# quadjr/aframe-gaussian-splatting

Measured on NVIDIA H100. Metric: frames/sec @1920x1080 (sort + splat raster, 1 M synthetic train-like splats), higher is better.
Workload: dtype f64 sort keys + f32 shading

## Files before the change

aframe-gaussian-splatting_b200/csrc/gs_sort.cu:

```cuda
#include <type_traits>

#include "gs_common.cuh"
#include "gs_depthkey.cuh"

namespace gs {

__device__ __forceinline__ bool worker_keep(const SortConsts &sc, const float4 c, const float s, double &depth) {
  const double x = c.x, y = c.y, z = c.z;
  depth = __dadd_rn(__dadd_rn(__dadd_rn(__dmul_rn(sc.view[0], x), __dmul_rn(sc.view[1], y)), __dmul_rn(sc.view[2], z)),
                    sc.view[3]);
  bool in_box = true;
  if (sc.has_cutout) {
    const double *e = sc.cutout;
    const double ny = -y;
    const double w = __ddiv_rn(
        1.0, __dadd_rn(__dadd_rn(__dadd_rn(__dmul_rn(e[3], x), __dmul_rn(e[7], ny)), __dmul_rn(e[11], z)), e[15]));
    const double c0 = __dmul_rn(
        __dadd_rn(__dadd_rn(__dadd_rn(__dmul_rn(e[0], x), __dmul_rn(e[4], ny)), __dmul_rn(e[8], z)), e[12]), w);
    const double c1 = __dmul_rn(
        __dadd_rn(__dadd_rn(__dadd_rn(__dmul_rn(e[1], x), __dmul_rn(e[5], ny)), __dmul_rn(e[9], z)), e[13]), w);
    const double c2 = __dmul_rn(
        __dadd_rn(__dadd_rn(__dadd_rn(__dmul_rn(e[2], x), __dmul_rn(e[6], ny)), __dmul_rn(e[10], z)), e[14]), w);
    if (c0 < -0.5 || c0 > 0.5 || c1 < -0.5 || c1 > 0.5 || c2 < -0.5 || c2 > 0.5) in_box = false;
  }
  return (depth < 0.0) && ((double)s > __dmul_rn(-0.0001, depth)) && in_box;
}

__global__ void __launch_bounds__(256) k_depth_cull(const float4 *__restrict__ cs, const float *__restrict__ sa,
                                                    const FrameParams *__restrict__ fp,
                                                    float *__restrict__ depth_out, FrameCounters *ctr) {
  GS_PDL_ENTRY();
  const SortConsts sc = fp->sc;
  const uint32_t n = fp->n_splats;
  double dmin = INFINITY, dmax = -INFINITY;
  uint32_t cnt = 0;
  const uint32_t stride = gridDim.x * blockDim.x;
  auto process = [&](uint32_t i, const float4 c, const float s) {
    double depth;
    const bool keep = worker_keep(sc, c, s, depth);
    float out = GS_DEPTH_REJECT;
    if (keep) {
      out = (float)depth;
      ++cnt;
      if (depth > dmax) dmax = depth;
      if (depth < dmin) dmin = depth;
    }
    depth_out[i] = out;
  };
  for (uint32_t i = blockIdx.x * blockDim.x + threadIdx.x; i < n; i += 2 * stride) {
    const uint32_t j = i + stride;
    const bool two = j < n;
    const float4 c0 = __ldg(cs + i);
    const float s0 = __ldg(sa + i);
    float4 c1 = c0;
    float s1 = s0;
    if (two) {
      c1 = __ldg(cs + j);
      s1 = __ldg(sa + j);
    }
    process(i, c0, s0);
    if (two) process(j, c1, s1);
  }
  for (int o = 16; o > 0; o >>= 1) {
    const double a = __shfl_xor_sync(0xffffffffu, dmin, o);
    const double b = __shfl_xor_sync(0xffffffffu, dmax, o);
    dmin = a < dmin ? a : dmin;
    dmax = b > dmax ? b : dmax;
    cnt += __shfl_xor_sync(0xffffffffu, cnt, o);
  }
  __shared__ double s_min[8], s_max[8];
  __shared__ uint32_t s_cnt[8];
  const int w = threadIdx.x >> 5, l = threadIdx.x & 31;
  if (l == 0) { s_min[w] = dmin; s_max[w] = dmax; s_cnt[w] = cnt; }
  __syncthreads();
  if (threadIdx.x == 0) {
    for (int k = 1; k < 8; ++k) {
      if (s_min[k] < dmin) dmin = s_min[k];
      if (s_max[k] > dmax) dmax = s_max[k];
      cnt += s_cnt[k];
    }
    if (cnt) {
      atomicMax(&ctr->sort.min_enc, ~enc_f64(dmin));
      atomicMax(&ctr->sort.max_enc, enc_f64(dmax));
      atomicAdd(&ctr->sort.n_valid, cnt);
    }
  }
}

__global__ void __launch_bounds__(256) k_depth_cull_scene(const float4 *__restrict__ cs, const float *__restrict__ sa,
                                                          const FrameParams *__restrict__ fp, const SceneTable *__restrict__ scene,
                                                          float *__restrict__ depth_out, FrameCounters *ctr, ObjCounters *octr) {
  GS_PDL_ENTRY();
  __shared__ uint32_t s_first[kMaxObjects], s_end[kMaxObjects], s_cnt[kMaxObjects];
  __shared__ unsigned long long s_min[kMaxObjects], s_max[kMaxObjects];
  const uint32_t n_obj = scene->n;
  for (uint32_t k = threadIdx.x; k < n_obj; k += blockDim.x) {
    s_first[k] = scene->obj[k].first;
    s_end[k] = scene->obj[k].end;
    s_cnt[k] = 0;
    s_min[k] = 0;
    s_max[k] = 0;
  }
  __syncthreads();
  const uint32_t n = fp->n_splats;
  const uint32_t stride = gridDim.x * blockDim.x;
  int cur = -1;
  double dmin = INFINITY, dmax = -INFINITY;
  uint32_t cnt = 0;
  auto flush = [&]() {
    if (cnt) {
      atomicMax(&s_min[cur], ~enc_f64(dmin));
      atomicMax(&s_max[cur], enc_f64(dmax));
      atomicAdd(&s_cnt[cur], cnt);
    }
    dmin = INFINITY;
    dmax = -INFINITY;
    cnt = 0;
  };
  auto process = [&](uint32_t i, const float4 c, const float s) {
    float out = GS_DEPTH_REJECT;
    const int k = scene_find(s_first, s_end, n_obj, i);
    double depth;
    if (k >= 0 && worker_keep(scene->obj[k].sc, c, s, depth)) {
      if (k != cur) {
        flush();
        cur = k;
      }
      out = (float)depth;
      ++cnt;
      if (depth > dmax) dmax = depth;
      if (depth < dmin) dmin = depth;
    }
    depth_out[i] = out;
  };
  for (uint32_t i = blockIdx.x * blockDim.x + threadIdx.x; i < n; i += 2 * stride) {
    const uint32_t j = i + stride;
    const bool two = j < n;
    const float4 c0 = __ldg(cs + i);
    const float s0 = __ldg(sa + i);
    float4 c1 = c0;
    float s1 = s0;
    if (two) {
      c1 = __ldg(cs + j);
      s1 = __ldg(sa + j);
    }
    process(i, c0, s0);
    if (two) process(j, c1, s1);
  }
  flush();
  __syncthreads();
  for (uint32_t k = threadIdx.x; k < n_obj; k += blockDim.x) {
    if (!s_cnt[k]) continue;
    atomicMax(&octr[k].min_enc, s_min[k]);
    atomicMax(&octr[k].max_enc, s_max[k]);
    atomicAdd(&octr[k].n_valid, s_cnt[k]);
    atomicMax(&ctr->sort.min_enc, s_min[k]);
    atomicMax(&ctr->sort.max_enc, s_max[k]);
    atomicAdd(&ctr->sort.n_valid, s_cnt[k]);
  }
}

template <bool IL>
__global__ void __launch_bounds__(256) k_scene_keys(const float *__restrict__ depth, const FrameParams *__restrict__ fp,
                                                    const SceneTable *__restrict__ scene, const ObjCounters *__restrict__ octr,
                                                    FrameCounters *ctr, uint32_t *__restrict__ key_out,
                                                    uint32_t *__restrict__ pay_out) {
  GS_PDL_ENTRY();
  __shared__ SceneKeyTable s_ent;
  __shared__ uint32_t s_in, s_drop;
  s_ent.load<IL>(scene, octr, ctr);
  if (threadIdx.x == 0) { s_in = 0; s_drop = 0; }
  __syncthreads();
  const uint32_t n = ctr->sort.n_valid ? fp->n_splats : 0u;
  uint32_t in = 0, drop = 0;
  for (uint32_t i = blockIdx.x * blockDim.x + threadIdx.x; i < n; i += gridDim.x * blockDim.x) {
    const float d = __ldg(depth + i);
    uint32_t key = kNoKey;
    if (d != GS_DEPTH_REJECT) {
      int k;
      key = s_ent.key<IL>(i, d, k);
      if (!IL && (key & 65536u)) {
        pay_out[i] = s_ent.first[k];
        ++drop;
      } else {
        pay_out[i] = i;
        ++in;
      }
    }
    key_out[i] = key;
  }
  for (int o = 16; o > 0; o >>= 1) {
    in += __shfl_xor_sync(0xffffffffu, in, o);
    drop += __shfl_xor_sync(0xffffffffu, drop, o);
  }
  if ((threadIdx.x & 31u) == 0) {
    if (in) atomicAdd(&s_in, in);
    if (drop) atomicAdd(&s_drop, drop);
  }
  __syncthreads();
  if (threadIdx.x == 0) {
    if (s_in) atomicAdd(&ctr->sort.n_inrange, s_in);
    if (s_drop) atomicAdd(&ctr->sort.n_dropped, s_drop);
  }
}

static int persistent_grid(gs_context *c, uint64_t n_elems, int per_cta, int ctas_per_sm) {
  uint64_t tiles = (n_elems + per_cta - 1) / per_cta;
  uint64_t cap = (uint64_t)c->sm_count * ctas_per_sm;
  if (tiles < 1) tiles = 1;
  return (int)(tiles < cap ? tiles : cap);
}

void launch_depth_cull(gs_context *c, const FrameParams *fp, FrameCounters *ctr, cudaStream_t st) {
  const int grid = persistent_grid(c, c->cap, 256 * 4, 8);
  launch_chain(c, k_depth_cull, grid, 256, st, c->center_scale, c->size_alpha, fp, c->depth, ctr);
}

void launch_depth_cull_scene(gs_context *c, const FrameParams *fp, const SceneTable *scene, ObjCounters *octr, FrameCounters *ctr,
                             cudaStream_t st) {
  const int grid = persistent_grid(c, c->cap, 256 * 4, 8);
  launch_chain(c, k_depth_cull_scene, grid, 256, st, c->center_scale, c->size_alpha, fp, scene, c->depth, ctr, octr);
}

void launch_scene_keys(gs_context *c, const FrameParams *fp, const SceneTable *scene, const ObjCounters *octr, FrameCounters *ctr,
                       bool interleave, cudaStream_t st) {
  const int grid = persistent_grid(c, c->cap, 256 * 4, 8);
  launch_chain(c, interleave ? k_scene_keys<true> : k_scene_keys<false>, grid, 256, st, (const float *)c->depth, fp, scene, octr,
               ctr, c->scene_key, c->scene_pay);
}

struct RadixScratch {
  uint32_t *table;
  uint32_t *totals;
  uint32_t stride;
};

struct RadixPass {
  using Carry = void;
  __device__ void prepare(uint32_t n) {}
  __device__ void hist_prologue(uint32_t n) const {}
  __device__ void hist_epilogue() {}
  __device__ void scanned(uint32_t total) const {}
  __device__ void digit_range(uint32_t d, uint32_t start, uint32_t end) const {}
};

template <class Pass>
__global__ void __launch_bounds__(kRadixThreads) k_radix_hist(Pass p, const RadixScratch s) {
  GS_PDL_ENTRY();
  __shared__ uint32_t h[256];
  const uint32_t tid = threadIdx.x, lane = tid & 31, warp = tid >> 5;
  const uint32_t n = p.count();
  const uint32_t num_chunks = (n + kRadixTile - 1) / kRadixTile;
  p.prepare(n);
  p.hist_prologue(n);
  for (uint32_t c = blockIdx.x; c < num_chunks; c += gridDim.x) {
    h[tid] = 0;
    __syncthreads();
    const uint32_t base = c * kRadixTile + warp * (32 * kRadixItems) + lane;
#pragma unroll
    for (int k = 0; k < kRadixItems; ++k) {
      const uint32_t i = base + k * 32;
      if (i < n) {
        uint32_t pay, carry;
        const uint32_t digit = p.load(i, pay, carry);
        if (digit != kInvalidDigit) atomicAdd(&h[digit], 1u);
      }
    }
    __syncthreads();
    s.table[(size_t)tid * s.stride + c] = h[tid];
    __syncthreads();
  }
  p.hist_epilogue();
}

template <class Pass>
__global__ void __launch_bounds__(256) k_radix_scan(const Pass p, const RadixScratch s) {
  GS_PDL_ENTRY();
  __shared__ uint32_t s_warp[8];
  __shared__ uint32_t s_carry;
  const uint32_t tid = threadIdx.x, lane = tid & 31, warp = tid >> 5;
  const uint32_t n = p.count();
  const uint32_t num_chunks = (n + kRadixTile - 1) / kRadixTile;
  uint32_t *row = s.table + (size_t)blockIdx.x * s.stride;
  if (tid == 0) s_carry = 0;
  __syncthreads();
  for (uint32_t b = 0; b < num_chunks; b += 256) {
    const uint32_t i = b + tid;
    const uint32_t v = (i < num_chunks) ? row[i] : 0u;
    uint32_t incl = v;
    for (int o = 1; o < 32; o <<= 1) {
      const uint32_t t = __shfl_up_sync(0xffffffffu, incl, o);
      if (lane >= (uint32_t)o) incl += t;
    }
    if (lane == 31) s_warp[warp] = incl;
    __syncthreads();
    uint32_t wbase = 0;
    for (uint32_t k = 0; k < warp; ++k) wbase += s_warp[k];
    const uint32_t carry = s_carry;
    if (i < num_chunks) row[i] = carry + wbase + incl - v;
    __syncthreads();
    if (tid == 255) s_carry = carry + wbase + incl;
    __syncthreads();
  }
  if (tid == 0) {
    s.totals[blockIdx.x] = s_carry;
    p.scanned(s_carry);
  }
}

constexpr int kScatThreads = 512;
constexpr int kScatItems = kRadixTile / kScatThreads;
constexpr int kScatWarps = kScatThreads / 32;

template <class Pass>
__global__ void __launch_bounds__(kScatThreads, 2) k_radix_scatter(Pass p, const RadixScratch s) {
  GS_PDL_ENTRY();
  constexpr bool kCarry = !std::is_void<typename Pass::Carry>::value;
  using carry_t = typename std::conditional<kCarry, typename Pass::Carry, uint8_t>::type;
  __shared__ uint32_t wcnt[kScatWarps][256];
  __shared__ uint32_t tile_off[256];
  __shared__ uint32_t s_loc[256];
  __shared__ uint32_t s_warp_tot[8];
  __shared__ uint32_t s_pay[kRadixTile];
  __shared__ carry_t s_carry[kCarry ? kRadixTile : 1];
  __shared__ uint8_t s_dig[kRadixTile];
  __shared__ uint32_t s_total;
  const uint32_t tid = threadIdx.x, lane = tid & 31, warp = tid >> 5;
  const uint32_t n = p.count();
  const uint32_t num_chunks = (n + kRadixTile - 1) / kRadixTile;
  if (blockIdx.x >= num_chunks) return;

  auto scan256 = [&](uint32_t v) -> uint32_t {
    uint32_t incl = v;
    for (int o = 1; o < 32; o <<= 1) {
      const uint32_t t = __shfl_up_sync(0xffffffffu, incl, o);
      if (lane >= (uint32_t)o) incl += t;
    }
    __syncthreads();
    if (lane == 31 && warp < 8) s_warp_tot[warp] = incl;
    __syncthreads();
    uint32_t wbase = 0;
    for (uint32_t k = 0; k < warp && k < 8; ++k) wbase += s_warp_tot[k];
    return wbase + incl - v;
  };

  const uint32_t dtot = tid < 256 ? s.totals[tid] : 0u;
  const uint32_t dbase = scan256(dtot);
  if (blockIdx.x == 0 && tid < 256) p.digit_range(tid, dbase, dbase + dtot);
  p.prepare(n);

  for (uint32_t c = blockIdx.x; c < num_chunks; c += gridDim.x) {
    const uint32_t toff = tid < 256 ? __ldg(s.table + (size_t)tid * s.stride + c) : 0u;
    for (uint32_t k = tid; k < kScatWarps * 256; k += kScatThreads) (&wcnt[0][0])[k] = 0u;
    const uint32_t base = c * kRadixTile + warp * (32 * kScatItems) + lane;
    uint32_t digit[kScatItems], pay[kScatItems], rank[kScatItems];
    carry_t carry[kScatItems];
#pragma unroll
    for (int k = 0; k < kScatItems; ++k) {
      const uint32_t i = base + k * 32;
      uint32_t cv = 0;
      digit[k] = kInvalidDigit;
      pay[k] = 0;
      if (i < n) digit[k] = p.load(i, pay[k], cv);
      carry[k] = (carry_t)cv;
    }
    __syncthreads();
#pragma unroll
    for (int k = 0; k < kScatItems; ++k) {
      const uint32_t d = digit[k];
      const uint32_t peers = __match_any_sync(0xffffffffu, d);
      const uint32_t lt = __popc(peers & ((1u << lane) - 1u));
      uint32_t prior = 0;
      if (d != kInvalidDigit) prior = wcnt[warp][d];
      __syncwarp();
      if (d != kInvalidDigit && lt == 0) wcnt[warp][d] = prior + __popc(peers);
      __syncwarp();
      rank[k] = prior + lt;
    }
    __syncthreads();
    uint32_t total = 0;
    if (tid < 256) {
#pragma unroll
      for (int w = 0; w < kScatWarps; ++w) {
        const uint32_t cnt = wcnt[w][tid];
        wcnt[w][tid] = total;
        total += cnt;
      }
    }
    const uint32_t loc = scan256(total);
    if (tid < 256) {
      s_loc[tid] = loc;
      tile_off[tid] = dbase + toff - loc;
      if (tid == 255) s_total = loc + total;
    }
    __syncthreads();
#pragma unroll
    for (int k = 0; k < kScatItems; ++k) {
      const uint32_t d = digit[k];
      if (d == kInvalidDigit) continue;
      const uint32_t lp = s_loc[d] + wcnt[warp][d] + rank[k];
      s_pay[lp] = pay[k];
      s_dig[lp] = (uint8_t)d;
      if (kCarry) s_carry[lp] = carry[k];
    }
    __syncthreads();
    const uint32_t nvalid = s_total;
    for (uint32_t i = tid; i < nvalid; i += kScatThreads)
      p.store(tile_off[s_dig[i]] + i, s_pay[i], kCarry ? (uint32_t)s_carry[i] : 0u);
    __syncthreads();
  }
}

template <class Pass>
static void run_pass(gs_context *c, const Pass &p, const RadixScratch &s, uint64_t n_max, cudaStream_t st) {
  const int grid = persistent_grid(c, n_max, kRadixTile, 8);
  launch_chain(c, k_radix_hist<Pass>, grid, kRadixThreads, st, p, s);
  launch_chain(c, k_radix_scan<Pass>, 256, 256, st, p, s);
  launch_chain(c, k_radix_scatter<Pass>, grid, kScatThreads, st, p, s);
}

struct D1 : RadixPass {
  using Carry = uint8_t;
  FrameCounters *ctr;
  const FrameParams *fp;
  const float *depth;
  uint32_t *idx_out; uint8_t *hi_out;
  DepthRange dr;
  uint32_t n_in, n_drop;
  __device__ uint32_t count() const { return ctr->sort.n_valid ? fp->n_splats : 0u; }
  __device__ void prepare(uint32_t n) { if (n) dr = load_depth_range(ctr); }
  __device__ uint32_t load(uint32_t i, uint32_t &pay, uint32_t &carry) {
    const float d = __ldg(depth + i);
    if (d == GS_DEPTH_REJECT) return kInvalidDigit;
    const int32_t key = depth_key(d, dr.min_depth, dr.depth_inv);
    if (key < 0 || key > 65535) { ++n_drop; return kInvalidDigit; }
    ++n_in;
    pay = i;
    carry = (uint32_t)key >> 8;
    return key & 255;
  }
  __device__ void store(uint32_t pos, uint32_t pay, uint32_t carry) const { idx_out[pos] = pay; hi_out[pos] = (uint8_t)carry; }
  __device__ void hist_epilogue() {
    __shared__ uint32_t s_in, s_drop;
    uint32_t in = n_in, drop = n_drop;
    for (int o = 16; o > 0; o >>= 1) {
      in += __shfl_xor_sync(0xffffffffu, in, o);
      drop += __shfl_xor_sync(0xffffffffu, drop, o);
    }
    if (threadIdx.x == 0) { s_in = 0; s_drop = 0; }
    __syncthreads();
    if ((threadIdx.x & 31u) == 0) { if (in) atomicAdd(&s_in, in); if (drop) atomicAdd(&s_drop, drop); }
    __syncthreads();
    if (threadIdx.x == 0) {
      if (s_in) atomicAdd(&ctr->sort.n_inrange, s_in);
      if (s_drop) atomicAdd(&ctr->sort.n_dropped, s_drop);
    }
  }
};

struct D2 : RadixPass {
  const FrameCounters *ctr;
  const uint8_t *dig; const uint32_t *idx;
  uint32_t *order;
  __device__ uint32_t count() const { return ctr->sort.n_inrange; }
  __device__ void hist_prologue(uint32_t n) const {
    const uint32_t nv = ctr->sort.n_valid;
    for (uint32_t j = n + blockIdx.x * blockDim.x + threadIdx.x; j < nv; j += gridDim.x * blockDim.x) order[j] = 0u;
  }
  __device__ uint32_t load(uint32_t i, uint32_t &pay, uint32_t &) const { pay = idx[i]; return dig[i]; }
  __device__ void store(uint32_t pos, uint32_t pay, uint32_t) const { order[pos] = pay; }
};

void launch_depth_radix(gs_context *c, const FrameParams *fp, FrameCounters *ctr, const FrameBufs &b, cudaStream_t st) {
  const RadixScratch s{c->table_n, c->totals, c->table_n_stride};
  run_pass(c, D1{{}, ctr, fp, c->depth, c->idx_a, c->dig_a}, s, c->cap, st);
  run_pass(c, D2{{}, ctr, c->dig_a, c->idx_a, b.order}, s, c->cap, st);
}

struct M1 : RadixPass {
  using Carry = uint16_t;
  const FrameCounters *ctr;
  const FrameParams *fp;
  const uint32_t *key, *pay_in;
  uint32_t *idx_out; uint16_t *hi_out;
  __device__ uint32_t count() const { return ctr->sort.n_valid ? fp->n_splats : 0u; }
  __device__ uint32_t load(uint32_t i, uint32_t &pay, uint32_t &carry) const {
    const uint32_t k = key[i];
    if (k == kNoKey) return kInvalidDigit;
    carry = k >> 8;
    pay = pay_in[i];
    return k & 255u;
  }
  __device__ void store(uint32_t pos, uint32_t pay, uint32_t carry) const { idx_out[pos] = pay; hi_out[pos] = (uint16_t)carry; }
};

struct M2 : RadixPass {
  using Carry = uint8_t;
  const FrameCounters *ctr;
  const uint16_t *hi; const uint32_t *idx;
  uint32_t *idx_out; uint8_t *hi_out;
  __device__ uint32_t count() const { return ctr->sort.n_valid; }
  __device__ uint32_t load(uint32_t i, uint32_t &pay, uint32_t &carry) const {
    const uint32_t h = hi[i];
    carry = h >> 8;
    pay = idx[i];
    return h & 255u;
  }
  __device__ void store(uint32_t pos, uint32_t pay, uint32_t carry) const { idx_out[pos] = pay; hi_out[pos] = (uint8_t)carry; }
};

struct M3 : RadixPass {
  const FrameCounters *ctr;
  const uint8_t *dig; const uint32_t *idx;
  uint32_t *order;
  __device__ uint32_t count() const { return ctr->sort.n_valid; }
  __device__ uint32_t load(uint32_t i, uint32_t &pay, uint32_t &) const { pay = idx[i]; return dig[i]; }
  __device__ void store(uint32_t pos, uint32_t pay, uint32_t) const { order[pos] = pay; }
};

void launch_scene_radix(gs_context *c, const FrameParams *fp, FrameCounters *ctr, const FrameBufs &b, cudaStream_t st) {
  const RadixScratch s{c->table_n, c->totals, c->table_n_stride};
  run_pass(c, M1{{}, ctr, fp, c->scene_key, c->scene_pay, c->idx_a, c->scene_hi}, s, c->cap, st);
  run_pass(c, M2{{}, ctr, c->scene_hi, c->idx_a, c->scene_pay, c->dig_a}, s, c->cap, st);
  run_pass(c, M3{{}, ctr, c->dig_a, c->scene_pay, b.order}, s, c->cap, st);
}

struct S1 : RadixPass {
  using Carry = uint8_t;
  const FrameCounters *ctr;
  const uint16_t *key; const uint32_t *idx;
  uint32_t *idx_out; uint8_t *hi_out;
  __device__ uint32_t count() const { return ctr->sort.n_valid; }
  __device__ uint32_t load(uint32_t i, uint32_t &pay, uint32_t &carry) const {
    const uint32_t k = key[i];
    carry = k >> 8;
    pay = idx[i];
    return k & 255u;
  }
  __device__ void store(uint32_t pos, uint32_t pay, uint32_t carry) const { idx_out[pos] = pay; hi_out[pos] = (uint8_t)carry; }
};

struct SM1 : RadixPass {
  using Carry = uint16_t;
  const FrameCounters *ctr;
  const SceneTable *scene;
  const uint32_t *key, *idx;
  uint32_t *idx_out; uint16_t *hi_out;
  __device__ uint32_t count() const { return ctr->sort.n_valid; }
  __device__ uint32_t load(uint32_t i, uint32_t &pay, uint32_t &carry) const {
    const uint32_t k = key[i];
    carry = k >> 8;
    pay = idx[i];
    if (k & 65536u) {
      uint32_t lo = 0, hi = scene->n;
      while (hi - lo > 1) {
        const uint32_t mid = (lo + hi) >> 1;
        if (scene->obj[mid].first <= pay) lo = mid; else hi = mid;
      }
      pay = scene->obj[lo].first;
    }
    return k & 255u;
  }
  __device__ void store(uint32_t pos, uint32_t pay, uint32_t carry) const { idx_out[pos] = pay; hi_out[pos] = (uint16_t)carry; }
};

struct SM1I : SM1 {
  __device__ uint32_t load(uint32_t i, uint32_t &pay, uint32_t &carry) const {
    const uint32_t k = key[i];
    carry = k >> 8;
    pay = idx[i];
    return k & 255u;
  }
};

void launch_slab_sort(gs_context *c, const FrameParams *fp, FrameCounters *ctr, const SceneTable *scene, bool interleave,
                      const FrameBufs &b, cudaStream_t st) {
  const RadixScratch s{c->table_n, c->totals, c->table_n_stride};
  if (scene) {
    const SM1 p1{{}, ctr, scene, c->scene_key, c->cidx, c->idx_a, c->scene_hi};
    if (interleave) run_pass(c, SM1I{p1}, s, c->cap, st);
    else run_pass(c, p1, s, c->cap, st);
    run_pass(c, M2{{}, ctr, c->scene_hi, c->idx_a, c->scene_pay, c->dig_a}, s, c->cap, st);
    run_pass(c, M3{{}, ctr, c->dig_a, c->scene_pay, b.order}, s, c->cap, st);
    return;
  }
  run_pass(c, S1{{}, ctr, c->ckey, c->cidx, c->idx_a, c->dig_a}, s, c->cap, st);
  run_pass(c, D2{{}, ctr, c->dig_a, c->idx_a, b.order}, s, c->cap, st);
}

__device__ __forceinline__ uint32_t f32_key(float d) { return ~__float_as_uint(d); }

__device__ __forceinline__ uint32_t scene_rank(const SceneTable *__restrict__ scene, uint32_t s) {
  uint32_t lo = 0, hi = scene->n;
  while (hi - lo > 1) {
    const uint32_t mid = (lo + hi) >> 1;
    if (scene->obj[mid].first <= s) lo = mid; else hi = mid;
  }
  return scene->obj[lo].rank;
}

constexpr int kRankDigit = -1;
template <int kShift, bool kAll>
struct Z : RadixPass {
  FrameCounters *ctr;
  const FrameParams *fp;
  const SceneTable *scene;
  const float *depth;
  const uint32_t *idx;
  uint32_t *idx_out;
  __device__ uint32_t count() const { return kAll ? (ctr->sort.n_valid ? fp->n_splats : 0u) : ctr->sort.n_valid; }
  __device__ uint32_t load(uint32_t i, uint32_t &pay, uint32_t &) const {
    const uint32_t s = kAll ? i : idx[i];
    pay = s;
    if constexpr (kShift == kRankDigit) {
      if (kAll && __ldg(depth + s) == GS_DEPTH_REJECT) return kInvalidDigit;
      return scene_rank(scene, s);
    } else {
      const float d = __ldg(depth + s);
      if (kAll && d == GS_DEPTH_REJECT) return kInvalidDigit;
      return (f32_key(d) >> kShift) & 255u;
    }
  }
  __device__ void store(uint32_t pos, uint32_t pay, uint32_t) const { idx_out[pos] = pay; }
  __device__ void scanned(uint32_t total) const {
    if (kAll && total) atomicAdd(&ctr->sort.n_inrange, total);
  }
};

template <bool kAll>
static void sort_f32(gs_context *c, const FrameParams *fp, FrameCounters *ctr, const SceneTable *scene, bool interleave,
                     const float *depth, const uint32_t *src, uint32_t *order, cudaStream_t st) {
  const RadixScratch s{c->table_n, c->totals, c->table_n_stride};
  uint32_t *a = c->idx_a, *b = c->scene_pay;
  if (scene && interleave) {
    run_pass(c, Z<kRankDigit, kAll>{{}, ctr, fp, scene, depth, src, a}, s, c->cap, st);
    run_pass(c, Z<0, false>{{}, ctr, fp, scene, depth, a, b}, s, c->cap, st);
    run_pass(c, Z<8, false>{{}, ctr, fp, scene, depth, b, a}, s, c->cap, st);
    run_pass(c, Z<16, false>{{}, ctr, fp, scene, depth, a, b}, s, c->cap, st);
    run_pass(c, Z<24, false>{{}, ctr, fp, scene, depth, b, order}, s, c->cap, st);
    return;
  }
  run_pass(c, Z<0, kAll>{{}, ctr, fp, scene, depth, src, a}, s, c->cap, st);
  run_pass(c, Z<8, false>{{}, ctr, fp, scene, depth, a, b}, s, c->cap, st);
  run_pass(c, Z<16, false>{{}, ctr, fp, scene, depth, b, a}, s, c->cap, st);
  if (!scene) {
    run_pass(c, Z<24, false>{{}, ctr, fp, scene, depth, a, order}, s, c->cap, st);
    return;
  }
  run_pass(c, Z<24, false>{{}, ctr, fp, scene, depth, a, b}, s, c->cap, st);
  run_pass(c, Z<kRankDigit, false>{{}, ctr, fp, scene, depth, b, order}, s, c->cap, st);
}

void launch_sort_f32(gs_context *c, const FrameParams *fp, FrameCounters *ctr, const SceneTable *scene, bool interleave,
                     const FrameBufs &b, cudaStream_t st) {
  sort_f32<true>(c, fp, ctr, scene, interleave, c->depth, nullptr, b.order, st);
}

void launch_slab_sort_f32(gs_context *c, FrameCounters *ctr, const SceneTable *scene, bool interleave, const float *zdepth,
                          const FrameBufs &b, cudaStream_t st) {
  sort_f32<false>(c, nullptr, ctr, scene, interleave, zdepth, c->cidx, b.order, st);
}

__device__ __forceinline__ void gather_record(const float4 *rec, float4 *inst_rec, uint32_t splat, uint32_t pos) {
  const float4 r0 = __ldg(rec + 2 * (size_t)splat);
  const float4 r1 = __ldg(rec + 2 * (size_t)splat + 1);
  inst_rec[2 * (size_t)pos] = r0;
  inst_rec[2 * (size_t)pos + 1] = r1;
}

struct T1 : RadixPass {
  using Carry = uint16_t;
  FrameCounters *ctr;
  const uint16_t *bin; const uint32_t *idx;
  uint16_t *bin_out; uint32_t *idx_out;
  const float4 *proj_rec; float4 *inst_rec; uint2 *bin_range;
  uint32_t n_bins;
  bool last;
  __device__ uint32_t count() const { return ctr->overflow ? 0u : (uint32_t)ctr->n_inst; }
  __device__ uint32_t load(uint32_t i, uint32_t &pay, uint32_t &carry) const {
    const uint16_t t = bin[i];
    if (t == kNoTile) return kInvalidDigit;
    carry = t;
    pay = idx[i];
    return t & 255;
  }
  __device__ void store(uint32_t pos, uint32_t pay, uint32_t carry) const {
    if (last) gather_record(proj_rec, inst_rec, pay, pos);
    else { idx_out[pos] = pay; bin_out[pos] = (uint16_t)carry; }
  }
  __device__ void scanned(uint32_t total) const { if (total) atomicAdd(&ctr->n_inst_kept, total); }
  __device__ void digit_range(uint32_t d, uint32_t start, uint32_t end) const {
    if (last && d < n_bins) bin_range[d] = make_uint2(start, end);
  }
};

struct T2 : RadixPass {
  using Carry = uint16_t;
  const FrameCounters *ctr;
  const uint16_t *bin; const uint32_t *idx;
  const float4 *proj_rec; float4 *inst_rec; uint16_t *bin_out;
  __device__ uint32_t count() const { return ctr->overflow ? 0u : ctr->n_inst_kept; }
  __device__ uint32_t load(uint32_t i, uint32_t &pay, uint32_t &carry) const {
    const uint16_t t = bin[i];
    carry = t;
    pay = idx[i];
    return (uint32_t)t >> 8;
  }
  __device__ void store(uint32_t pos, uint32_t pay, uint32_t carry) const {
    gather_record(proj_rec, inst_rec, pay, pos);
    bin_out[pos] = (uint16_t)carry;
  }
};

__global__ void __launch_bounds__(256) k_tile_ranges(const uint16_t *__restrict__ tile_f, FrameCounters *ctr,
                                                     uint2 *__restrict__ range) {
  GS_PDL_ENTRY();
  const uint32_t n = ctr->overflow ? 0u : ctr->n_inst_kept;
  for (uint32_t i = blockIdx.x * blockDim.x + threadIdx.x; i < n; i += gridDim.x * blockDim.x) {
    const uint32_t t = tile_f[i];
    if (i == 0 || tile_f[i - 1] != t) range[t].x = i;
    if (i == n - 1 || tile_f[i + 1] != t) range[t].y = i + 1;
  }
}

struct ViewRecs {
  const float4 *rec_x;
  uint32_t x_stride;
  uint32_t base1, base2, base3;
  __device__ __forceinline__ const float4 *of(const float4 *rec0, uint32_t bin) const {
    const uint32_t v = (bin >= base1 ? 1u : 0u) + (bin >= base2 ? 1u : 0u) + (bin >= base3 ? 1u : 0u);
    return v ? rec_x + 2 * (size_t)(v - 1) * x_stride : rec0;
  }
};
struct T1S : T1 {
  ViewRecs vr;
  __device__ void store(uint32_t pos, uint32_t pay, uint32_t carry) const {
    if (last) gather_record(vr.of(proj_rec, carry), inst_rec, pay, pos);
    else { idx_out[pos] = pay; bin_out[pos] = (uint16_t)carry; }
  }
};
struct T2S : T2 {
  ViewRecs vr;
  __device__ void store(uint32_t pos, uint32_t pay, uint32_t carry) const {
    gather_record(vr.of(proj_rec, carry), inst_rec, pay, pos);
    bin_out[pos] = (uint16_t)carry;
  }
};

struct T1P : T1 {
  uint32_t *pay_out;
  __device__ void store(uint32_t pos, uint32_t pay, uint32_t carry) const {
    if (last) { gather_record(proj_rec, inst_rec, pay, pos); pay_out[pos] = pay; }
    else { idx_out[pos] = pay; bin_out[pos] = (uint16_t)carry; }
  }
};
struct T2P : T2 {
  uint32_t *pay_out;
  __device__ void store(uint32_t pos, uint32_t pay, uint32_t carry) const {
    gather_record(proj_rec, inst_rec, pay, pos);
    pay_out[pos] = pay;
    bin_out[pos] = (uint16_t)carry;
  }
};

void launch_tile_radix_pick(gs_context *c, FrameCounters *ctr, const FrameBufs &b, uint32_t n_bins, uint32_t *pay, cudaStream_t st) {
  const RadixScratch s{c->table_d, c->totals + 256, c->table_d_stride};
  const bool last = n_bins <= 256u;
  const T1 t1{{}, ctr, c->inst_tile, c->inst_idx, c->inst_tile_b, c->inst_idx_b, b.proj_rec, b.inst_rec, b.bin_range, n_bins, last};
  run_pass(c, T1P{t1, pay}, s, c->cap_inst, st);
  if (last) return;
  const T2 t2{{}, ctr, c->inst_tile_b, c->inst_idx_b, b.proj_rec, b.inst_rec, c->inst_tile_f};
  run_pass(c, T2P{t2, pay}, s, c->cap_inst, st);
  launch_chain(c, k_tile_ranges, persistent_grid(c, c->cap_inst, 256 * 8, 8), 256, st, (const uint16_t *)c->inst_tile_f, ctr,
               b.bin_range);
}

void launch_tile_radix(gs_context *c, FrameCounters *ctr, const FrameBufs &b, uint32_t n_bins, cudaStream_t st) {
  const RadixScratch s{c->table_d, c->totals + 256, c->table_d_stride};
  const bool last = n_bins <= 256u;
  if (b.views) {
    static_assert(kMaxViews == 4, "ViewRecs holds three bases");
    const ViewRecs vr{b.proj_recx, b.x_stride, b.bin_base[1], b.bin_base[2], b.bin_base[3]};
    const T1 t1{{}, ctr, c->inst_tile, c->inst_idx, c->inst_tile_b, c->inst_idx_b, b.proj_rec, b.inst_rec, b.bin_range, n_bins, last};
    run_pass(c, T1S{t1, vr}, s, c->cap_inst, st);
    if (last) return;
    const T2 t2{{}, ctr, c->inst_tile_b, c->inst_idx_b, b.proj_rec, b.inst_rec, c->inst_tile_f};
    run_pass(c, T2S{t2, vr}, s, c->cap_inst, st);
    launch_chain(c, k_tile_ranges, persistent_grid(c, c->cap_inst, 256 * 8, 8), 256, st, (const uint16_t *)c->inst_tile_f, ctr,
                 b.bin_range);
    return;
  }
  run_pass(c, T1{{}, ctr, c->inst_tile, c->inst_idx, c->inst_tile_b, c->inst_idx_b, b.proj_rec, b.inst_rec, b.bin_range, n_bins, last},
           s, c->cap_inst, st);
  if (last) return;
  run_pass(c, T2{{}, ctr, c->inst_tile_b, c->inst_idx_b, b.proj_rec, b.inst_rec, c->inst_tile_f}, s, c->cap_inst, st);
  launch_chain(c, k_tile_ranges, persistent_grid(c, c->cap_inst, 256 * 8, 8), 256, st, (const uint16_t *)c->inst_tile_f, ctr,
               b.bin_range);
}

template <int kShift>
struct P : RadixPass {
  const uint32_t *key, *perm;
  uint32_t *perm_out;
  uint32_t n;
  __device__ uint32_t count() const { return n; }
  __device__ uint32_t load(uint32_t i, uint32_t &pay, uint32_t &) const {
    const uint32_t row = kShift == 0 ? i : perm[i];
    pay = row;
    return (__ldg(key + row) >> kShift) & 255u;
  }
  __device__ void store(uint32_t pos, uint32_t pay, uint32_t) const { perm_out[pos] = pay; }
};

uint32_t *launch_ply_sort(gs_context *c, const uint32_t *key, uint32_t *perm_a, uint32_t *perm_b, uint32_t *table,
                          uint32_t *totals, uint32_t n, cudaStream_t st) {
  const RadixScratch s{table, totals, (n + kRadixTile - 1) / kRadixTile + 1};
  run_pass(c, P<0>{{}, key, nullptr, perm_a, n}, s, n, st);
  run_pass(c, P<8>{{}, key, perm_a, perm_b, n}, s, n, st);
  run_pass(c, P<16>{{}, key, perm_b, perm_a, n}, s, n, st);
  run_pass(c, P<24>{{}, key, perm_a, perm_b, n}, s, n, st);
  return perm_b;
}

}
```

Before: 3027.

## Vectorize depth cull, restructure radix scan/scatter, and branchless depth key

The depth-cull kernel now processes four splats per thread, using float4 loads for opacity and float4 stores for depth, with a tail handled by block 0. The radix histogram hoists loads ahead of the shared-memory atomics and uses a no-bounds-check path for full tiles. The scan kernel gives each warp one digit row and has each lane scan 8 entries, which removes block-level syncs. The scatter kernel pads the per-warp count table to avoid bank conflicts, replaces the serial per-digit warp-count loop with parallel segmented shuffles, fuses two 256-wide scans into one, packs digit and carry into one register, and unrolls stores by two. D1's depth-key conversion becomes a branchless bit-level JS ToInt32; this risks subtle numerical differences from the original depth_key.

```diff
diff --git a/aframe-gaussian-splatting_b200/csrc/gs_sort.cu b/aframe-gaussian-splatting_b200/csrc/gs_sort.cu
--- a/aframe-gaussian-splatting_b200/csrc/gs_sort.cu
+++ b/aframe-gaussian-splatting_b200/csrc/gs_sort.cu
@@ -35,7 +35,7 @@
   double dmin = INFINITY, dmax = -INFINITY;
   uint32_t cnt = 0;
   const uint32_t stride = gridDim.x * blockDim.x;
-  auto process = [&](uint32_t i, const float4 c, const float s) {
+  auto process = [&](const float4 c, const float s) -> float {
     double depth;
     const bool keep = worker_keep(sc, c, s, depth);
     float out = GS_DEPTH_REJECT;
@@ -45,21 +45,22 @@
       if (depth > dmax) dmax = depth;
       if (depth < dmin) dmin = depth;
     }
-    depth_out[i] = out;
+    return out;
   };
-  for (uint32_t i = blockIdx.x * blockDim.x + threadIdx.x; i < n; i += 2 * stride) {
-    const uint32_t j = i + stride;
-    const bool two = j < n;
-    const float4 c0 = __ldg(cs + i);
-    const float s0 = __ldg(sa + i);
-    float4 c1 = c0;
-    float s1 = s0;
-    if (two) {
-      c1 = __ldg(cs + j);
-      s1 = __ldg(sa + j);
-    }
-    process(i, c0, s0);
-    if (two) process(j, c1, s1);
+  const uint32_t n4 = n & ~3u;
+  for (uint32_t i = (blockIdx.x * blockDim.x + threadIdx.x) * 4u; i < n4; i += stride * 4u) {
+    const float4 c0 = __ldg(cs + i), c1 = __ldg(cs + i + 1), c2 = __ldg(cs + i + 2), c3 = __ldg(cs + i + 3);
+    const float4 s = __ldg((const float4 *)(sa + i));
+    float4 out;
+    out.x = process(c0, s.x);
+    out.y = process(c1, s.y);
+    out.z = process(c2, s.z);
+    out.w = process(c3, s.w);
+    *(float4 *)(depth_out + i) = out;
+  }
+  if (blockIdx.x == 0 && threadIdx.x < n - n4) {
+    const uint32_t i = n4 + threadIdx.x;
+    depth_out[i] = process(__ldg(cs + i), __ldg(sa + i));
   }
   for (int o = 16; o > 0; o >>= 1) {
     const double a = __shfl_xor_sync(0xffffffffu, dmin, o);
@@ -255,17 +256,25 @@
   p.hist_prologue(n);
   for (uint32_t c = blockIdx.x; c < num_chunks; c += gridDim.x) {
     h[tid] = 0;
-    __syncthreads();
     const uint32_t base = c * kRadixTile + warp * (32 * kRadixItems) + lane;
-#pragma unroll
-    for (int k = 0; k < kRadixItems; ++k) {
-      const uint32_t i = base + k * 32;
-      if (i < n) {
-        uint32_t pay, carry;
-        const uint32_t digit = p.load(i, pay, carry);
-        if (digit != kInvalidDigit) atomicAdd(&h[digit], 1u);
+    uint32_t digit[kRadixItems];
+    auto load_slice = [&](auto tail) {
+#pragma unroll
+      for (int k = 0; k < kRadixItems; ++k) {
+        const uint32_t i = base + k * 32;
+        digit[k] = kInvalidDigit;
+        if (!decltype(tail)::value || i < n) {
+          uint32_t pay, carry;
+          digit[k] = p.load(i, pay, carry);
+        }
       }
-    }
+    };
+    if ((c + 1) * kRadixTile <= n) load_slice(std::false_type{});
+    else load_slice(std::true_type{});
+    __syncthreads();
+#pragma unroll
+    for (int k = 0; k < kRadixItems; ++k)
+      if (digit[k] != kInvalidDigit) atomicAdd(&h[digit[k]], 1u);
     __syncthreads();
     s.table[(size_t)tid * s.stride + c] = h[tid];
     __syncthreads();
@@ -273,54 +282,59 @@
   p.hist_epilogue();
 }
 
+constexpr int kScanRows = 8;
+constexpr int kScanSpan = 8;
+
 template <class Pass>
-__global__ void __launch_bounds__(256) k_radix_scan(const Pass p, const RadixScratch s) {
+__global__ void __launch_bounds__(32 * kScanRows) k_radix_scan(const Pass p, const RadixScratch s) {
   GS_PDL_ENTRY();
-  __shared__ uint32_t s_warp[8];
-  __shared__ uint32_t s_carry;
-  const uint32_t tid = threadIdx.x, lane = tid & 31, warp = tid >> 5;
+  const uint32_t lane = threadIdx.x & 31, digit = blockIdx.x * kScanRows + (threadIdx.x >> 5);
   const uint32_t n = p.count();
   const uint32_t num_chunks = (n + kRadixTile - 1) / kRadixTile;
-  uint32_t *row = s.table + (size_t)blockIdx.x * s.stride;
-  if (tid == 0) s_carry = 0;
-  __syncthreads();
-  for (uint32_t b = 0; b < num_chunks; b += 256) {
-    const uint32_t i = b + tid;
-    const uint32_t v = (i < num_chunks) ? row[i] : 0u;
-    uint32_t incl = v;
+  uint32_t *row = s.table + (size_t)digit * s.stride;
+  uint32_t carry = 0;
+  for (uint32_t b = 0; b < num_chunks; b += 32 * kScanSpan) {
+    const uint32_t first = b + lane * kScanSpan;
+    uint32_t v[kScanSpan], sum = 0;
+#pragma unroll
+    for (int k = 0; k < kScanSpan; ++k) {
+      v[k] = first + k < num_chunks ? row[first + k] : 0u;
+      sum += v[k];
+    }
+    uint32_t incl = sum;
+#pragma unroll
     for (int o = 1; o < 32; o <<= 1) {
       const uint32_t t = __shfl_up_sync(0xffffffffu, incl, o);
       if (lane >= (uint32_t)o) incl += t;
     }
-    if (lane == 31) s_warp[warp] = incl;
-    __syncthreads();
-    uint32_t wbase = 0;
-    for (uint32_t k = 0; k < warp; ++k) wbase += s_warp[k];
-    const uint32_t carry = s_carry;
-    if (i < num_chunks) row[i] = carry + wbase + incl - v;
-    __syncthreads();
-    if (tid == 255) s_carry = carry + wbase + incl;
-    __syncthreads();
-  }
-  if (tid == 0) {
-    s.totals[blockIdx.x] = s_carry;
-    p.scanned(s_carry);
+    uint32_t run = carry + incl - sum;
+#pragma unroll
+    for (int k = 0; k < kScanSpan; ++k) {
+      if (first + k < num_chunks) row[first + k] = run;
+      run += v[k];
+    }
+    carry += __shfl_sync(0xffffffffu, incl, 31);
+  }
+  if (lane == 0) {
+    s.totals[digit] = carry;
+    p.scanned(carry);
   }
 }
 
 constexpr int kScatThreads = 512;
 constexpr int kScatItems = kRadixTile / kScatThreads;
 constexpr int kScatWarps = kScatThreads / 32;
+constexpr int kWcntPitch = 257;
 
 template <class Pass>
 __global__ void __launch_bounds__(kScatThreads, 2) k_radix_scatter(Pass p, const RadixScratch s) {
   GS_PDL_ENTRY();
   constexpr bool kCarry = !std::is_void<typename Pass::Carry>::value;
   using carry_t = typename std::conditional<kCarry, typename Pass::Carry, uint8_t>::type;
-  __shared__ uint32_t wcnt[kScatWarps][256];
+  __shared__ uint32_t wcnt[kScatWarps * kWcntPitch];
   __shared__ uint32_t tile_off[256];
   __shared__ uint32_t s_loc[256];
-  __shared__ uint32_t s_warp_tot[8];
+  __shared__ uint32_t s_warp_tot[2][8];
   __shared__ uint32_t s_pay[kRadixTile];
   __shared__ carry_t s_carry[kCarry ? kRadixTile : 1];
   __shared__ uint8_t s_dig[kRadixTile];
@@ -330,83 +344,110 @@
   const uint32_t num_chunks = (n + kRadixTile - 1) / kRadixTile;
   if (blockIdx.x >= num_chunks) return;
 
-  auto scan256 = [&](uint32_t v) -> uint32_t {
-    uint32_t incl = v;
+  auto scan256x2 = [&](uint32_t &a, uint32_t &b) {
+    uint32_t ia = a, ib = b;
+#pragma unroll
     for (int o = 1; o < 32; o <<= 1) {
-      const uint32_t t = __shfl_up_sync(0xffffffffu, incl, o);
-      if (lane >= (uint32_t)o) incl += t;
-    }
-    __syncthreads();
-    if (lane == 31 && warp < 8) s_warp_tot[warp] = incl;
-    __syncthreads();
-    uint32_t wbase = 0;
-    for (uint32_t k = 0; k < warp && k < 8; ++k) wbase += s_warp_tot[k];
-    return wbase + incl - v;
+      const uint32_t ta = __shfl_up_sync(0xffffffffu, ia, o), tb = __shfl_up_sync(0xffffffffu, ib, o);
+      if (lane >= (uint32_t)o) { ia += ta; ib += tb; }
+    }
+    if (lane == 31 && warp < 8) { s_warp_tot[0][warp] = ia; s_warp_tot[1][warp] = ib; }
+    __syncthreads();
+    uint32_t wa = 0, wb = 0;
+    for (uint32_t k = 0; k < warp && k < 8; ++k) { wa += s_warp_tot[0][k]; wb += s_warp_tot[1][k]; }
+    a = wa + ia - a;
+    b = wb + ib - b;
   };
 
   const uint32_t dtot = tid < 256 ? s.totals[tid] : 0u;
-  const uint32_t dbase = scan256(dtot);
-  if (blockIdx.x == 0 && tid < 256) p.digit_range(tid, dbase, dbase + dtot);
   p.prepare(n);
 
   for (uint32_t c = blockIdx.x; c < num_chunks; c += gridDim.x) {
     const uint32_t toff = tid < 256 ? __ldg(s.table + (size_t)tid * s.stride + c) : 0u;
-    for (uint32_t k = tid; k < kScatWarps * 256; k += kScatThreads) (&wcnt[0][0])[k] = 0u;
     const uint32_t base = c * kRadixTile + warp * (32 * kScatItems) + lane;
-    uint32_t digit[kScatItems], pay[kScatItems], rank[kScatItems];
-    carry_t carry[kScatItems];
+    uint32_t key[kScatItems], pay[kScatItems], rank[kScatItems];
+    auto load_slice = [&](auto tail) {
+#pragma unroll
+      for (int k = 0; k < kScatItems; ++k) {
+        const uint32_t i = base + k * 32;
+        uint32_t cv = 0;
+        key[k] = kInvalidDigit;
+        pay[k] = 0;
+        if (!decltype(tail)::value || i < n) {
+          const uint32_t d = p.load(i, pay[k], cv);
+          if (d != kInvalidDigit) key[k] = d | (kCarry ? (uint32_t)(carry_t)cv << 8 : 0u);
+        }
+      }
+    };
+    if ((c + 1) * kRadixTile <= n) load_slice(std::false_type{});
+    else load_slice(std::true_type{});
+    for (uint32_t k = tid; k < kScatWarps * kWcntPitch; k += kScatThreads) wcnt[k] = 0u;
+    __syncthreads();
+    uint32_t *const my_cnt = wcnt + warp * kWcntPitch;
 #pragma unroll
     for (int k = 0; k < kScatItems; ++k) {
-      const uint32_t i = base + k * 32;
-      uint32_t cv = 0;
-      digit[k] = kInvalidDigit;
-      pay[k] = 0;
-      if (i < n) digit[k] = p.load(i, pay[k], cv);
-      carry[k] = (carry_t)cv;
-    }
-    __syncthreads();
-#pragma unroll
-    for (int k = 0; k < kScatItems; ++k) {
-      const uint32_t d = digit[k];
+      const uint32_t d = key[k] == kInvalidDigit ? kInvalidDigit : key[k] & 255u;
       const uint32_t peers = __match_any_sync(0xffffffffu, d);
       const uint32_t lt = __popc(peers & ((1u << lane) - 1u));
       uint32_t prior = 0;
-      if (d != kInvalidDigit) prior = wcnt[warp][d];
+      if (d != kInvalidDigit) prior = my_cnt[d];
       __syncwarp();
-      if (d != kInvalidDigit && lt == 0) wcnt[warp][d] = prior + __popc(peers);
+      if (d != kInvalidDigit && lt == 0) my_cnt[d] = prior + __popc(peers);
       __syncwarp();
       rank[k] = prior + lt;
     }
     __syncthreads();
-    uint32_t total = 0;
+    {
+      const uint32_t w = lane & 15;
+#pragma unroll
+      for (int r = 0; r < 8; ++r) {
+        const uint32_t d = 32 * (warp >> 1) + 8 * (warp & 1) + r + 16 * (lane >> 4);
+        const uint32_t v = wcnt[w * kWcntPitch + d];
+        uint32_t incl = v;
+#pragma unroll
+        for (int o = 1; o < 16; o <<= 1) {
+          const uint32_t t = __shfl_up_sync(0xffffffffu, incl, o, 16);
+          if (w >= (uint32_t)o) incl += t;
+        }
+        wcnt[w * kWcntPitch + d] = incl - v;
+        if (w == 15) s_loc[d] = incl;
+      }
+    }
+    __syncthreads();
+    const uint32_t cnt = tid < 256 ? s_loc[tid] : 0u;
+    uint32_t loc = cnt, dbase = dtot;
+    scan256x2(loc, dbase);
     if (tid < 256) {
-#pragma unroll
-      for (int w = 0; w < kScatWarps; ++w) {
-        const uint32_t cnt = wcnt[w][tid];
-        wcnt[w][tid] = total;
-        total += cnt;
-      }
-    }
-    const uint32_t loc = scan256(total);
-    if (tid < 256) {
+      if (c == 0) p.digit_range(tid, dbase, dbase + dtot);
       s_loc[tid] = loc;
       tile_off[tid] = dbase + toff - loc;
-      if (tid == 255) s_total = loc + total;
+      if (tid == 255) s_total = loc + cnt;
     }
     __syncthreads();
 #pragma unroll
     for (int k = 0; k < kScatItems; ++k) {
-      const uint32_t d = digit[k];
-      if (d == kInvalidDigit) continue;
-      const uint32_t lp = s_loc[d] + wcnt[warp][d] + rank[k];
+      if (key[k] == kInvalidDigit) continue;
+      const uint32_t d = key[k] & 255u;
+      const uint32_t lp = s_loc[d] + my_cnt[d] + rank[k];
       s_pay[lp] = pay[k];
       s_dig[lp] = (uint8_t)d;
-      if (kCarry) s_carry[lp] = carry[k];
+      if (kCarry) s_carry[lp] = (carry_t)(key[k] >> 8);
     }
     __syncthreads();
     const uint32_t nvalid = s_total;
-    for (uint32_t i = tid; i < nvalid; i += kScatThreads)
-      p.store(tile_off[s_dig[i]] + i, s_pay[i], kCarry ? (uint32_t)s_carry[i] : 0u);
+    for (uint32_t i = tid; i < nvalid; i += 2 * kScatThreads) {
+      const uint32_t j = i + kScatThreads;
+      const bool two = j < nvalid;
+      const uint32_t pos0 = tile_off[s_dig[i]] + i, pay0 = s_pay[i], car0 = kCarry ? (uint32_t)s_carry[i] : 0u;
+      uint32_t pos1 = 0, pay1 = 0, car1 = 0;
+      if (two) {
+        pos1 = tile_off[s_dig[j]] + j;
+        pay1 = s_pay[j];
+        car1 = kCarry ? (uint32_t)s_carry[j] : 0u;
+      }
+      p.store(pos0, pay0, car0);
+      if (two) p.store(pos1, pay1, car1);
+    }
     __syncthreads();
   }
 }
@@ -415,8 +456,16 @@
 static void run_pass(gs_context *c, const Pass &p, const RadixScratch &s, uint64_t n_max, cudaStream_t st) {
   const int grid = persistent_grid(c, n_max, kRadixTile, 8);
   launch_chain(c, k_radix_hist<Pass>, grid, kRadixThreads, st, p, s);
-  launch_chain(c, k_radix_scan<Pass>, 256, 256, st, p, s);
+  launch_chain(c, k_radix_scan<Pass>, 256 / kScanRows, 32 * kScanRows, st, p, s);
   launch_chain(c, k_radix_scatter<Pass>, grid, kScatThreads, st, p, s);
+}
+
+__device__ __forceinline__ int32_t js_to_int32_flat(double q) {
+  const unsigned long long b = (unsigned long long)__double_as_longlong(q);
+  const int e = (int)((b >> 52) & 0x7FFu) - 1075;
+  const unsigned long long m = (b & 0xFFFFFFFFFFFFFull) | 0x10000000000000ull;
+  const uint32_t lo = e >= 32 ? 0u : e >= 0 ? (uint32_t)(m << e) : e > -53 ? (uint32_t)(m >> -e) : 0u;
+  return (int32_t)((b >> 63) ? 0u - lo : lo);
 }
 
 struct D1 : RadixPass {
@@ -431,13 +480,14 @@
   __device__ void prepare(uint32_t n) { if (n) dr = load_depth_range(ctr); }
   __device__ uint32_t load(uint32_t i, uint32_t &pay, uint32_t &carry) {
     const float d = __ldg(depth + i);
-    if (d == GS_DEPTH_REJECT) return kInvalidDigit;
-    const int32_t key = depth_key(d, dr.min_depth, dr.depth_inv);
-    if (key < 0 || key > 65535) { ++n_drop; return kInvalidDigit; }
-    ++n_in;
+    const bool kept = d != GS_DEPTH_REJECT;
+    const int32_t key = js_to_int32_flat(__dmul_rn(__dsub_rn((double)d, dr.min_depth), dr.depth_inv));
+    const bool in = key >= 0 && key <= 65535;
+    n_drop += kept && !in;
+    n_in += kept && in;
     pay = i;
     carry = (uint32_t)key >> 8;
-    return key & 255;
+    return kept && in ? (uint32_t)key & 255u : kInvalidDigit;
   }
   __device__ void store(uint32_t pos, uint32_t pay, uint32_t carry) const { idx_out[pos] = pay; hi_out[pos] = (uint8_t)carry; }
   __device__ void hist_epilogue() {
```

Measured after the change: 3149 (median of 6 runs). +4.1%, better.
